# Sweetroll97/GaussianProcessPathModelling

Measured on AMD Instinct MI355X. Metric: gp_fit_predict_points_per_sec, higher is better.
Workload: dtype f64; 1 GPU; C3: exact GP fit+predict, N=65536 d=3 rbf float64, M=4096, inputs resident in HBM; N=65536, d=3, M=4096, kernel=rbf, block=2048, parallelism=1 gpu

## Files before the change

### gaussianprocesspathmodelling_amd/csrc/gpx_api.hip

```cpp
#include <hip/hip_runtime.h>
#include <dlfcn.h>

#include <algorithm>
#include <climits>
#include <cmath>
#include <cstdio>
#include <cstdlib>
#include <cstring>
#include <new>
#include <string>
#include <vector>

#include "../../include/gpx.h"
#include "gpx_cov.h"
#include "gpx_env.h"
#include "gpx_internal.h"

using namespace gpx;

namespace {

thread_local std::string g_create_error;

#define GPX_CATCH_ALL                                  \
  catch (const std::bad_alloc&) { return GPX_E_NOMEM; } \
  catch (...) { return GPX_E_HIP; }

constexpr int RHS_ROWS = 64;

struct Phase {
  hipEvent_t a, b;
  double* target;
};

struct DevBuf {
  void* p = nullptr;
  size_t cap = 0;
  DevBuf() = default;
  DevBuf(DevBuf&& o) noexcept : p(o.p), cap(o.cap) { o.p = nullptr, o.cap = 0; }
  DevBuf& operator=(DevBuf&& o) noexcept {
    std::swap(p, o.p);
    std::swap(cap, o.cap);
    return *this;
  }
  ~DevBuf() {
    if (p) (void)hipFree(p);
  }
};

struct Comm;
struct Group;

}

struct gpx_handle {
  gpx_config cfg{};
  int nb = 1024;
  int nb_solve = 256;
  int nb_pred = 1024;
  EnvKnobs env;
  hipStream_t st = nullptr;
  hipStream_t st2 = nullptr;
  hipStream_t st3 = nullptr;
  hipStream_t st4 = nullptr;
  hipStream_t st5 = nullptr;
  std::string err;
  gpx_timings tm{};
  bool fitted = false;
  int64_t N = 0, Npad = 0, ld = 0, ldp = 0;
  int d = 0, k = 0, n_ls = 1;
  double sf2 = 0, sn2 = 0, jitter = 0;
  double logdet = 0;
  DevBuf X, Xs, ls, K, Winv, P, YT, Y, scalars, info;
  DevBuf var, meanout;
  struct ScratchBufs {
    DevBuf Q, Qs, VT, MT;
    DevBuf Tsol;
    DevBuf MTpart;
    DevBuf ZT, gpart;
    DevBuf ZTloc, ZTpack;
    DevBuf Sv;
// ... 247 lines not shown
    if (seq == 0) HIPCHK(h, hipMemsetAsync(dflag, 0, sizeof(unsigned), s));
    HIPCHK(h, hipEventRecord(e0, s));
    HIPCHK(h, hipStreamWaitEvent(iw->aux, e0, 0));
    HIPCHK(h, hipMemsetAsync(iw->U, 0, (size_t)iw->nbw * iw->ldu * sizeof(T), iw->aux));
    launch_set_diag_one_t<T>(iw->U, iw->ldu, nbp, iw->aux);
    HIPCHK(h, hipMemsetAsync(Wp, 0, (size_t)iw->nbw * iw->nbw * sizeof(T), iw->aux));
  }
  const int diag_step = h->env.diag_step;
  const int nq = nbp / KB;
  for (int q = 0; q < nq;) {
    const int w = (diag_step == 128 && q + 1 < nq) ? 2 : 1;
    const int64_t oq = o + (int64_t)q * KB;
    T* Aqq = A + oq * ld + oq;
    T* Wq = Winv + (oq / KB) * (KB * KB);
    seq += 2;
    if (w == 2)
      launch_potf2_128<T>(Aqq, ld, Wq, gidx0 + oq, info, s, iw && use_flag ? dflag : nullptr, seq);
    else
      launch_potf2_64<T>(Aqq, ld, Wq, gidx0 + oq, info, s, iw && use_flag ? dflag : nullptr, seq);
    const int64_t rem = o + nbp - (oq + w * KB);
    if (rem > 0) {
      T* panel = A + (oq + w * KB) * ld + oq;
      launch_trsm_rlt<T>(panel, ld, rem, Aqq, ld, Wq, w * KB, nullptr, 0, s);
      launch_gemm_nt<T>(64, A + (oq + w * KB) * ld + (oq + w * KB), ld, panel, ld, panel, ld, rem, rem, w * KB, 1, 0, s);
    }
    if (iw) {
      if (use_flag) {
        if (q > 0) {
          launch_wait_counter(dflag, seq - 1, info, iw->aux);
          launch_inv_extend<T>(iw->U, iw->ldu, A + o * ld + o, ld, Winv + (o / KB) * (KB * KB), q, q + w, Wp,
                               iw->nbw, iw->aux, 1);
        }
        launch_wait_counter(dflag, seq, info, iw->aux);
      } else {
        if (int rc = stream_waits(h, iw->aux, s, "block inverse")) return rc;
        launch_inv_extend<T>(iw->U, iw->ldu, A + o * ld + o, ld, Winv + (o / KB) * (KB * KB), q, q + w, Wp, iw->nbw,
                             iw->aux, 1);
      }
      launch_inv_extend<T>(iw->U, iw->ldu, A + o * ld + o, ld, Winv + (o / KB) * (KB * KB), q, q + w, Wp, iw->nbw,
                           iw->aux, 2);
    }
    q += w;
  }
  if (iw) {
    iw->seq = seq;
    if (int rc = record_event(h, iw->aux, "block inverse", &iw->ready)) return rc;
  }
  return GPX_OK;
}

template <typename T>
int panel_solve_enqueue(gpx_handle* h, T* A, int64_t ld, int64_t o, int nbp, int64_t rows_main, int64_t nx,
                        const T* Winv, T* P, int64_t ldp, hipStream_t s, InvWork<T>* iw, int set, int64_t row0 = 0,
                        hipEvent_t prev = nullptr, bool last = true) {
  T* Apanel = A + (o + nbp + row0) * ld + o;
  P += row0 * ldp;
  const int64_t rows = rows_main + nx;
  if (rows <= 0) {
    if (iw && last && row0 > 0) {
      if (int rc = record_event(h, h->st4, "panel copy", &iw->copied[set])) return rc;
    }
    return GPX_OK;
  }
  if (!iw) {
    launch_trsm_rlt<T>(Apanel, ld, rows, A + o * ld + o, ld, Winv + (o / KB) * (KB * KB), nbp, P, ldp, s);
    return GPX_OK;
  }
  const T* Wp = iw->W + (o / iw->nbw) * (int64_t)iw->nbw * iw->nbw;
  HIPCHK(h, hipStreamWaitEvent(s, iw->ready, 0));
  if (row0 == 0 && last) prev = iw->copied[set];
  if (prev) HIPCHK(h, hipStreamWaitEvent(s, prev, 0));
  const int tile_main = gemm_nt_tile((rows_main % 128 == 0 && nbp % 128 == 0) ? 128 : 64, rows_main, nbp, 4);
  if (rows_main > 0 && nx > 0 && tile_main == 64) {
    launch_gemm_nt_fixed<T>(64, P, ldp, Apanel, ld, Wp, iw->nbw, rows, nbp, nbp, 4, 1, s);
  } else {
    if (rows_main > 0) launch_gemm_nt_fixed<T>(tile_main, P, ldp, Apanel, ld, Wp, iw->nbw, rows_main, nbp, nbp, 4, 1, s);
    if (nx > 0)
      launch_gemm_nt<T>(64, P + rows_main * ldp, ldp, Apanel + rows_main * ld, ld, Wp, iw->nbw, nx, nbp, nbp, 4, 1,
                        s);
  }
  if (int rc = stream_waits(h, h->st4, s, "panel copy")) return rc;
  launch_copy2d<T>(Apanel, ld, P, ldp, rows, nbp, h->st4);
  if (last) return record_event(h, h->st4, "panel copy", &iw->copied[set]);
  return GPX_OK;
}

template <typename T>
int chol_enqueue(gpx_handle* h, T* A, int64_t ld, int64_t n, int nb, T* Winv, T* P0, T* P1,
                 int64_t ldp, int* info, int64_t gidx0, bool profile, int64_t nx = 0,
                 InvWork<T>* iw = nullptr, int64_t nx_side = 0) {
  hipStream_t s0 = h->st, s1 = h->st2;
  T* Pbuf[2] = {P0, P1};
  int rc;
  const EnvKnobs& env = h->env;
  const bool fuse_env = fused_strip_in_force(h);
  unsigned* ctr = reinterpret_cast<unsigned*>(info + 8);
  unsigned target = 0;
  auto is_fused = [&](int64_t o) -> bool {
    if (!fuse_env || o >= n) return false;
    const int nbp = (int)std::min<int64_t>(nb, n - o);
    const int64_t ntrail = n - (o + nbp);
    if (ntrail <= 0) return false;
    const int nbn = (int)std::min<int64_t>(nb, ntrail);
    const int64_t nrest = ntrail - nbn;
    if (nrest <= 0 || ntrail % 128 != 0 || nbn % 128 != 0) return false;
    return gemm_nt_tile(128, nrest, nrest, 1) == 128 && gemm_nt_tile(128, ntrail, nbn, 2) == 128;
  };
  auto bordered_update = [&](int64_t o, const T* Pc, hipStream_t s) {
    const int nbp = (int)std::min<int64_t>(nb, n - o);
    const int64_t t0 = o + nbp, ntrail = n - t0;
    if (nx <= 0 || ntrail <= 0) return;
    launch_gemm_nt<T>(nx % 128 == 0 && ntrail % 128 == 0 ? 128 : 64, A + n * ld + t0, ld, Pc + ntrail * ldp, ldp, Pc,
                      ldp, nx, ntrail, nbp, 0, 0, s);
  };
  auto bordered_block = [&](int64_t o, const T* Pc, hipStream_t s, int64_t c0, int64_t nc, int64_t r0, int64_t nr) {
    const int nbp = (int)std::min<int64_t>(nb, n - o);
    const int64_t t0 = o + nbp, ntrail = n - t0;
    if (nr <= 0 || nc <= 0) return;
    launch_gemm_nt<T>(nr % 128 == 0 && nc % 128 == 0 ? 128 : 64, A + (n + r0) * ld + c0, ld, Pc + (ntrail + r0) * ldp, ldp,
                      Pc + (c0 - t0) * ldp, ldp, nr, nc, nbp, 0, 0, s);
  };
  auto update_is_big = [&](int64_t o) -> bool {
    if (o >= n) return false;
    const int nbp = (int)std::min<int64_t>(nb, n - o);
    const int64_t ntrail = n - (o + nbp);
    if (ntrail <= 0) return false;
    const int nbn = (int)std::min<int64_t>(nb, ntrail);
    const int64_t nrest = ntrail - nbn;
    return nrest > 0 && ntrail % 128 == 0 && nbn % 128 == 0 && gemm_nt_tile(128, nrest, nrest, 1) == 128;
  };
  const bool split_env = split_strip_in_force(h);
  const bool top_env = env.solve_top;
  const int rest_split = env.rest_split;
  const int64_t nxs = split_env ? nx_side : 0, nxc = nx - nxs;
  auto side_solve = [&](int64_t o, T* Pp, hipStream_t s) -> int {
    if (nxs <= 0) return GPX_OK;
    const int nbp = (int)std::min<int64_t>(nb, n - o);
    T* Aside = A + (n + nxc) * ld + o;
    T* Pside = Pp + ((n - o - nbp) + nxc) * ldp;
    if (!iw) {
      launch_trsm_rlt<T>(Aside, ld, nxs, A + o * ld + o, ld, Winv + (o / KB) * (KB * KB), nbp, Pside, ldp, s);
      return GPX_OK;
    }
    HIPCHK(h, hipStreamWaitEvent(s, iw->ready, 0));
    launch_gemm_nt<T>(nxs % 128 == 0 && nbp % 128 == 0 ? 128 : 64, Pside, ldp, Aside, ld,
                      iw->W + (o / iw->nbw) * (int64_t)iw->nbw * iw->nbw, iw->nbw, nxs, nbp, nbp, 4, 1, s);
    launch_copy2d<T>(Aside, ld, Pside, ldp, nxs, nbp, s);
    return GPX_OK;
  };
  LatencyGuard latency_guard;
  set_latency_mode(1);
  const int resv_k = env.cu_self_reserve;
  ReserveGuard reserve_guard;
  if (resv_k > 0 && split_env) {
    if ((rc = ensure(h, h->resv_ring, (size_t)RESV_RING * 8 * sizeof(unsigned)))) return rc;
    HIPCHK(h, hipMemsetAsync(h->resv_ring.p, 0, (size_t)RESV_RING * 8 * sizeof(unsigned), s0));
    reserve_ring((unsigned*)h->resv_ring.p, RESV_RING, env.resv_form);
  }
  const bool any_fused = is_fused(0);
  if (any_fused) HIPCHK(h, hipMemsetAsync(ctr, 0, sizeof(unsigned), s0));
  {
    const int nb0 = (int)std::min<int64_t>(nb, n);
    {
      PhaseScope ps(h, &h->tm.chol_diag, profile);
      if ((rc = diag_enqueue(h, A, ld, 0, nb0, Winv, info, gidx0, s0, iw))) return rc;
    }
    {
      PhaseScope ps(h, &h->tm.chol_trsm, profile);
      if ((rc = panel_solve_enqueue(h, A, ld, 0, nb0, n - nb0, nxc, Winv, Pbuf[0], ldp, s0, iw, 0))) return rc;
    }
    if (any_fused) {
      bordered_update(0, Pbuf[0], s0);
      if ((rc = stream_waits(h, s1, s0, "look-ahead"))) return rc;
    }
  }
  hipEvent_t e_main = nullptr;
  if (split_env && n > nb && (rc = record_event(h, s0, "look-ahead", &e_main))) return rc;
  int step = 0;
  for (int64_t o = 0; o < n; o += nb, ++step) {
    const int nbp = (int)std::min<int64_t>(nb, n - o);
    const int64_t t0 = o + nbp;
    const int64_t ntrail = n - t0;
    if (ntrail <= 0) {
      if ((rc = side_solve(o, Pbuf[step & 1], s0))) return rc;
      break;
    }
    T* Pc = Pbuf[step & 1];
    T* Pn = Pbuf[(step + 1) & 1];
    const int nbn = (int)std::min<int64_t>(nb, ntrail);
    const int64_t nrest = ntrail - nbn;
    const int tile = (ntrail % 128 == 0 && nbn % 128 == 0) ? 128 : 64;
    hipEvent_t e_panel = next_event(h);
    if (!e_panel) return fail(h, GPX_E_HIP, "hipEventCreate failed (look-ahead)");
    set_latency_mode(update_is_big(o) ? 0 : 1);
    if (is_fused(o)) {
      {
        PhaseScope ps(h, &h->tm.chol_syrk, profile);
        target += launch_gemm_nt_fused<T>(A + t0 * ld + t0, ld, Pc, ldp, ntrail, nbn, nbp, ctr, s0);
        h->tm.syrk_flops += (double)ntrail * (double)(ntrail + 1) * (double)nbp;
        h->tm.syrk_launches += 1;
      }
      launch_wait_counter(ctr, target, info, s1);
      {
        PhaseScope ps(h, &h->tm.chol_diag, profile, s1);
        if ((rc = diag_enqueue(h, A, ld, t0, nbn, Winv, info, gidx0, s1, iw))) return rc;
      }
      {
        PhaseScope ps(h, &h->tm.chol_trsm, profile, s1);
        if ((rc = panel_solve_enqueue(h, A, ld, t0, nbn, nrest, nx, Winv, Pn, ldp, s1, iw, (step + 1) & 1))) return rc;
      }
      HIPCHK(h, hipEventRecord(e_panel, s1));
      if (is_fused(t0)) bordered_update(t0, Pn, s1);
      HIPCHK(h, hipStreamWaitEvent(s0, e_panel, 0));
      continue;
    }
    if (split_env) {
      hipStream_t sm = s0;
      const int resv_it = (resv_k > 0 && (env.resv_all || ntrail <= (int64_t)(rest_split + 1) * nb)) ? resv_k : 0;
      if (e_main) HIPCHK(h, hipStreamWaitEvent(s1, e_main, 0));
      {
        PhaseScope ps(h, &h->tm.chol_strip, profile, s1);
        launch_gemm_nt<T>(tile, A + t0 * ld + t0, ld, Pc, ldp, Pc, ldp, nbn, nbn, nbp, 1, 0, s1);
      }
      set_reserve_mode(resv_it);
      {
        PhaseScope ps(h, &h->tm.chol_strip, profile, sm);
        if (nrest > 0)
          launch_gemm_nt<T>(tile, A + (t0 + nbn) * ld + t0, ld, Pc + (int64_t)nbn * ldp, ldp, Pc, ldp, nrest, nbn, nbp, 0,
                            0, sm);
        bordered_block(o, Pc, sm, t0, nbn, 0, nxc);
      }
      hipEvent_t e_below;
      if ((rc = record_event(h, sm, "look-ahead", &e_below))) return rc;
      const int nbn2 = (int)std::min<int64_t>(nb, nrest);
      const bool ahead = nrest > nbn2 && nrest <= (int64_t)rest_split * nb;
      T* Cr = A + (t0 + nbn) * ld + (t0 + nbn);
      const T* Pr = Pc + (int64_t)nbn * ldp;
      if (ahead) {
        {
          PhaseScope ps(h, &h->tm.chol_strip, profile, sm);
          launch_gemm_nt<T>(tile, Cr, ld, Pr, ldp, Pr, ldp, nrest, nbn2, nbp, 2, 0, sm);
        }
        if ((rc = record_event(h, sm, "look-ahead", &e_main))) return rc;
      }
      const int64_t nr = ahead ? nrest - nbn2 : nrest, off = ahead ? nbn2 : 0;
      if (nr > 0) {
        const bool big = gemm_nt_tile(tile, nr, nr, 1) == 128;
        PhaseScope ps(h, big ? &h->tm.chol_syrk : &h->tm.chol_strip, profile, sm);
        launch_gemm_nt<T>(tile, Cr + off * ld + off, ld, Pr + off * ldp, ldp, Pr + off * ldp, ldp, nr, nr, nbp, 1, 0, sm);
        if (big) {
          h->tm.syrk_flops += (double)nr * (double)(nr + 1) * (double)nbp;
          h->tm.syrk_launches += 1;
        }
      }
      if (!ahead && (rc = record_event(h, sm, "look-ahead", &e_main))) return rc;
      {
        PhaseScope ps(h, &h->tm.chol_strip, profile, sm);
        bordered_block(o, Pc, sm, t0 + nbn, nrest, 0, nxc);
        if ((rc = side_solve(o, Pc, sm))) return rc;
        bordered_block(o, Pc, sm, t0, ntrail, nxc, nxs);
      }
      set_reserve_mode(0);
      {
        PhaseScope ps(h, &h->tm.chol_diag, profile, s1);
        set_reserve_chain(resv_it > 0 ? env.resv_chain : 0);
        rc = diag_enqueue(h, A, ld, t0, nbn, Winv, info, gidx0, s1, iw);
        set_reserve_chain(0);
        if (rc) return rc;
      }
      HIPCHK(h, hipStreamWaitEvent(s1, e_below, 0));
      const int64_t top = (iw && top_env) ? std::min<int64_t>(nrest, nb) : nrest;
      hipEvent_t prev_copied = iw ? iw->copied[(step + 1) & 1] : nullptr;
      {
        PhaseScope ps(h, &h->tm.chol_trsm, profile, s1);
        if (top < nrest || (iw && top_env)) {
          if ((rc = panel_solve_enqueue(h, A, ld, t0, nbn, top, 0, Winv, Pn, ldp, s1, iw, (step + 1) & 1, 0, prev_copied,
                                        false)))
            return rc;
        } else if ((rc = panel_solve_enqueue(h, A, ld, t0, nbn, nrest, nxc, Winv, Pn, ldp, s1, iw, (step + 1) & 1))) {
          return rc;
        }
      }
      HIPCHK(h, hipEventRecord(e_panel, s1));
      HIPCHK(h, hipStreamWaitEvent(sm, e_panel, 0));
      if (top < nrest || (iw && top_env)) {
        PhaseScope ps(h, &h->tm.chol_trsm, profile, sm);
        set_reserve_mode(resv_it);
        rc = panel_solve_enqueue(h, A, ld, t0, nbn, nrest - top, nxc, Winv, Pn, ldp, sm, iw, (step + 1) & 1, top, prev_copied,
                                 true);
        set_reserve_mode(0);
        if (rc) return rc;
      }
      continue;
    }
    {
      PhaseScope ps(h, &h->tm.chol_strip, profile);
      set_latency_mode(1);
      launch_gemm_nt<T>(tile, A + t0 * ld + t0, ld, Pc, ldp, Pc, ldp, ntrail, nbn, nbp, 2, 0, s0);
      set_latency_mode(update_is_big(o) ? 0 : 1);
      bordered_update(o, Pc, s0);
    }
    if ((rc = stream_waits(h, s1, s0, "look-ahead"))) return rc;
    {
      {
        PhaseScope ps(h, &h->tm.chol_diag, profile, s1);
        if ((rc = diag_enqueue(h, A, ld, t0, nbn, Winv, info, gidx0, s1, iw))) return rc;
      }
      {
        PhaseScope ps(h, &h->tm.chol_trsm, profile, s1);
        if ((rc = panel_solve_enqueue(h, A, ld, t0, nbn, nrest, nx, Winv, Pn, ldp, s1, iw, (step + 1) & 1))) return rc;
      }
    }
    HIPCHK(h, hipEventRecord(e_panel, s1));
    if (nrest > 0) {
      const bool big = gemm_nt_tile(tile, nrest, nrest, 1) == 128;
      PhaseScope ps(h, big ? &h->tm.chol_syrk : &h->tm.chol_strip, profile);
      launch_gemm_nt<T>(tile, A + (t0 + nbn) * ld + (t0 + nbn), ld, Pc + (int64_t)nbn * ldp, ldp,
                        Pc + (int64_t)nbn * ldp, ldp, nrest, nrest, nbp, 1, 0, s0);
      if (big) {
        h->tm.syrk_flops += (double)nrest * (double)(nrest + 1) * (double)nbp;
        h->tm.syrk_launches += 1;
      }
    }
    HIPCHK(h, hipStreamWaitEvent(s0, e_panel, 0));
  }
  if (iw) {
    for (hipStream_t sj : {iw->aux, h->st4})
      if ((rc = stream_waits(h, s0, sj, "join"))) return rc;
  }
  return GPX_OK;
}

template <typename T>
struct SolveWork {
  const T* W = nullptr;
  int nbw = 0;
  T *T0 = nullptr, *T1 = nullptr;
  int64_t ldt = 0;
};

template <typename T>
int solve_fwd_enqueue(gpx_handle* h, T* XT, int64_t rows, const T* L, int64_t ld, int64_t n, int nb,
                      const T* Winv, const SolveWork<T>* wb = nullptr) {
  hipStream_t s0 = h->st, s1 = h->st2;
  const int tile = (rows % 128 == 0) ? 128 : 64;
  LatencyGuard latency_guard;
  set_latency_mode(1);
  if (rows < 128 || !s1) {
    for (int64_t o = 0; o < n; o += nb) {
      const int nbp = (int)std::min<int64_t>(nb, n - o);
      launch_trsm_rlt<T>(XT + o, ld, rows, L + o * ld + o, ld, Winv + (o / KB) * (KB * KB), nbp, nullptr,
                         0, s0);
      const int64_t ntrail = n - (o + nbp);
      if (ntrail > 0)
        launch_gemm_nt<T>((ntrail % 128 == 0) ? tile : 64, XT + o + nbp, ld, XT + o, ld,
                          L + (o + nbp) * ld + o, ld, rows, ntrail, nbp, 0, 0, s0);
    }
    return GPX_OK;
  }
  const bool dense = wb && wb->nbw == nb && wb->T0 && h->st4;
  T* Ts[2] = {dense ? wb->T0 : nullptr, dense ? wb->T1 : nullptr};
  hipEvent_t e_copy[2] = {nullptr, nullptr};
  const int64_t ldt = dense ? wb->ldt : 0;
// ... 143 lines not shown

template <typename T>
int dense_solve_work(gpx_handle* h, DevBuf& buf, int64_t rows, SolveWork<T>* sw) {
  if (h->nbw != h->nb_pred || (h->comm && !h->repl)) return GPX_OK;
  int rc;
  sw->ldt = h->nbw + ld_skew<T>();
  if ((rc = ensure(h, buf, (size_t)2 * rows * sw->ldt * sizeof(T)))) return rc;
  sw->W = (const T*)h->Wblk.p;
  sw->nbw = h->nbw;
  sw->T0 = (T*)buf.p;
  sw->T1 = sw->T0 + rows * sw->ldt;
  return GPX_OK;
}

template <typename T>
void mean_product(gpx_handle* h, T* MT, int64_t ldm, const T* rhsT, const T* VT, int64_t cols, T* part, int64_t ldpart) {
  const int ksplit = splitk_splits(h->Npad);
  if (ksplit > 1)
    launch_gemm_nt_splitk<T>(MT, ldm, rhsT, h->ld, VT, h->ld, RHS_ROWS, cols, h->Npad, ksplit, part, ldpart, h->st);
  else
    launch_gemm_nt<T>(64, MT, ldm, rhsT, h->ld, VT, h->ld, RHS_ROWS, cols, h->Npad, 0, 1, h->st);
}

template <typename T>
int ensure_mean_partials(gpx_handle* h, DevBuf& part, int64_t ldpart) {
  const int ksplit = splitk_splits(h->Npad);
  return ksplit > 1 ? ensure(h, part, (size_t)ksplit * RHS_ROWS * ldpart * sizeof(T)) : GPX_OK;
}

template <typename T>
void bordered_mean_var(gpx_handle* h, const T* VT, int64_t rows, int64_t rows_pad, int64_t ldm, bool want_var) {
  {
    PhaseScope ps(h, &h->tm.mean);
    mean_product<T>(h, (T*)h->scr.MT.p, ldm, (const T*)h->zT, VT, rows_pad, (T*)h->scr.MTpart.p, ldm);
    launch_unpack_rhs<T>((const T*)h->scr.MT.p, ldm, rows, h->k, 1.0, (T*)h->meanout.p, h->st);
  }
  if (want_var) {
    PhaseScope ps(h, &h->tm.var);
    launch_var_rows<T>(VT, h->ld, rows, h->Npad, h->sf2, (T*)h->var.p, h->st);
  }
}

template <typename T>
int deliver_mean_var(gpx_handle* h, void* mean, void* var, int64_t M, int32_t mem_kind) {
  PhaseScope ps(h, &h->tm.d2h);
  int rc;
  if ((rc = copy_out(h, mean, h->meanout.p, (size_t)M * h->k * sizeof(T), mem_kind))) return rc;
  return var ? copy_out(h, var, h->var.p, (size_t)M * sizeof(T), mem_kind) : GPX_OK;
}

template <typename T>
int predict_core(gpx_handle* h, const void* Xq, int64_t M, bool want_var, int32_t mem_kind);
bool few_solver_applies(const gpx_handle* h);
template <typename T>
int solve_few(gpx_handle* h, T* RT, int k, const T* L, int64_t ld, int64_t n, const T* W, int nb, bool forward = true,
              bool backward = true);

}

#include "gpx_shard.inc"
#include "gpx_group.inc"

namespace {

template <typename T>
int stage_fit_weights(gpx_handle* h, int64_t N, int64_t cap) {
  h->weighted = false;
  if (h->nw_set == 0) return GPX_OK;
  int rc;
  if ((rc = ensure(h, h->Wfit, (size_t)cap * sizeof(T)))) return rc;
  if (h->cfg.dtype == GPX_MIXED) {
    if ((rc = ensure(h, h->Wfit64, (size_t)cap * 8))) return rc;
    HIPCHK(h, hipMemcpyAsync(h->Wfit64.p, h->Wset.p, (size_t)N * 8, hipMemcpyDeviceToDevice, h->st));
    launch_f64_to_f32((const double*)h->Wfit64.p, (float*)h->Wfit.p, N, h->st);
  } else {
    HIPCHK(h, hipMemcpyAsync(h->Wfit.p, h->Wset.p, (size_t)N * sizeof(T), hipMemcpyDeviceToDevice, h->st));
  }
  h->weighted = true;
  return GPX_OK;
}

template <typename T>
int fit_impl(gpx_handle* h, const void* X, const void* y, int64_t N, int32_t d, int32_t k,
             const double* lengthscale, int32_t n_ls, double sf2, double sn2, double jitter,
             int32_t mem_kind, int64_t* info, const void* Xq = nullptr, int64_t M = 0, bool retried = false) {
  const int64_t Npad = round_up(N, TILE);
  const int64_t Mpad = Xq ? round_up(M, TILE) : 0;
  const int64_t cap = h->reserve > 0 ? std::max(Npad, round_up(h->reserve, TILE)) : Npad;
  const int64_t capN = h->reserve > 0 ? cap : N;
  const int64_t ld = cap + ld_skew<T>();
  if (h->cfg.block == 0) {
    h->nb = auto_panel_width(h, Npad);
    if (h->env.nb_pred < 0) h->nb_pred = h->nb;
  }
  const int64_t ldp = h->nb + ld_skew<T>();
  h->N = N; h->Npad = Npad; h->ld = ld; h->ldp = ldp; h->d = d; h->k = k; h->n_ls = n_ls;
  h->sf2 = sf2; h->sn2 = sn2; h->jitter = jitter;
  const bool profile = (h->cfg.flags & GPX_FLAG_PROFILE) != 0;
  gpx_timings& tm = h->tm;
  tm.h2d = tm.kbuild = tm.chol = tm.solve = tm.logdet = tm.fit_total = 0;
  tm.chol_diag = tm.chol_trsm = tm.chol_strip = tm.chol_syrk = tm.syrk_flops = tm.comm = 0;
  tm.syrk_launches = 0;
  tm.kbuild_bytes = (double)sizeof(T) * ((double)N * (double)(N + 1) / 2.0 + (double)N * d);

  int rc;
  if ((rc = flag_handover_probe(h))) return rc;
  if ((rc = ensure(h, h->X, (size_t)capN * d * sizeof(T)))) return rc;
  if ((rc = ensure(h, h->Y, (size_t)capN * k * sizeof(T)))) return rc;
  if ((rc = ensure(h, h->Xs, (size_t)cap * d * sizeof(T)))) return rc;
  if ((rc = ensure(h, h->ls, MAX_D * 8))) return rc;
  const int64_t NX = RHS_ROWS + Mpad;
  if (Xq && (rc = ensure_queries<T>(h, M))) return rc;
  if ((rc = ensure(h, h->K, (size_t)(cap + NX) * ld * sizeof(T)))) return rc;
  if ((rc = ensure(h, h->Winv, (size_t)(cap / KB) * KB * KB * sizeof(T)))) return rc;
  if ((rc = ensure(h, h->P, (size_t)2 * (cap + NX) * ldp * sizeof(T)))) return rc;
  if ((rc = ensure(h, h->scalars, 64))) return rc;
  if ((rc = ensure(h, h->info, 64))) return rc;
  const int64_t nblk = (cap + h->nb - 1) / h->nb;
  const int64_t ldu = h->nb + ld_skew<T>();
  if ((rc = ensure(h, h->Wblk, (size_t)nblk * h->nb * h->nb * sizeof(T)))) return rc;
  if ((rc = ensure(h, h->Ublk, (size_t)h->nb * ldu * sizeof(T)))) return rc;
  if ((rc = stage_fit_weights<T>(h, N, cap))) return rc;
  InvWork<T> iw;
  iw.W = (T*)h->Wblk.p;
  iw.U = (T*)h->Ublk.p;
  iw.ldu = ldu;
  iw.nbw = h->nb;
  iw.aux = h->st3;
  h->nbw = 0;

  T* dK = (T*)h->K.p;
  h->Lfac = dK;
  h->repl = false;
  T* dYT = dK + Npad * ld;
  h->zT = dYT;
  h->alphaT = nullptr;
  h->alpha_ready = false;
  int* dInfo = (int*)h->info.p;
  {
    PhaseScope total(h, &tm.fit_total);
    {
      PhaseScope ps(h, &tm.h2d);
      if ((rc = copy_in(h, h->X.p, X, (size_t)N * d * sizeof(T), mem_kind))) return rc;
      if ((rc = copy_in(h, h->Y.p, y, (size_t)N * k * sizeof(T), mem_kind))) return rc;
      if ((rc = copy_in(h, h->ls.p, lengthscale, (size_t)n_ls * 8, GPX_MEM_HOST))) return rc;
      const int init = INT_MAX;
      HIPCHK(h, hipMemcpyAsync(dInfo, &init, sizeof(int), hipMemcpyHostToDevice, h->st));
    }
    {
      PhaseScope ps(h, &tm.kbuild);
      launch_scale_points<T>((const T*)h->X.p, N, Npad, d, (const double*)h->ls.p, n_ls,
                          (T*)h->Xs.p, h->st);
      if (h->weighted)
        launch_kbuild_sym_w<T>(h->cfg.kernel, (const T*)h->Xs.p, N, Npad, d, sf2, (const T*)h->Wfit.p, sn2, jitter, dK, ld,
                               h->st);
      else
        launch_kbuild_sym<T>(h->cfg.kernel, (const T*)h->Xs.p, N, Npad, d, sf2, sn2 + jitter, dK, ld, h->st);
      if (Xq) {
        if ((rc = upload_queries<T>(h, Xq, M, mem_kind))) return rc;
        launch_kbuild_cross<T>(h->cfg.kernel, (const T*)h->scr.Qs.p, M, Mpad, (const T*)h->Xs.p, N, Npad, d, sf2,
                            dK + (Npad + RHS_ROWS) * ld, ld, h->st);
      }
    }
    {
      PhaseScope ps(h, &tm.chol);
      launch_pack_rhs<T>((const T*)h->Y.p, N, k, dYT, ld, Npad, RHS_ROWS, h->st);
      if ((rc = chol_enqueue<T>(h, dK, ld, Npad, h->nb, (T*)h->Winv.p, (T*)h->P.p,
                                (T*)h->P.p + (Npad + NX) * ldp, ldp, dInfo, 0, profile, NX, &iw, Mpad)))
        return rc;
    }
    {
      PhaseScope ps(h, &tm.logdet);
      launch_logdet<T>(dK, ld, Npad, (double*)h->scalars.p, h->st);
    }
  }
  int hinfo = 0;
  HIPCHK(h, hipMemcpyAsync(&hinfo, dInfo, sizeof(int), hipMemcpyDeviceToHost, h->st));
  HIPCHK(h, hipMemcpyAsync(&h->logdet, h->scalars.p, sizeof(double), hipMemcpyDeviceToHost, h->st));
  if ((rc = finish_call(h))) return rc;
  if (hinfo < 0) {
    if (retry_with_events(h, retried))
      return fit_impl<T>(h, X, y, N, d, k, lengthscale, n_ls, sf2, sn2, jitter, mem_kind, info, Xq, M, true);
    return fail(h, GPX_E_HIP,
                "a stream parked on a device flag timed out: kernels are being serialised across streams — "
                "set GPX_CHAIN_FLAG=0 (and leave GPX_FUSED_STRIP unset) to hand over by hipEvents instead");
  }
  tm.handover_flags = chain_flag_enabled(h) ? 1.0 : 0.0;
  tm.handover_retries = (double)h->flag_retries;
  *info = (hinfo == INT_MAX) ? 0 : (int64_t)hinfo;
  h->fitted = (*info == 0);
  if (h->fitted) h->nbw = h->nb;
  return GPX_OK;
}


template <typename T>
int append_room(gpx_handle* h, int64_t Nnew, bool with_weights) {
  const int64_t skew = ld_skew<T>(), cap0 = h->ld - skew, NpadNew = round_up(Nnew, TILE), want = round_up(h->reserve, TILE);
  const int64_t N = h->N, Npad = h->Npad, nb = h->nb, d = h->d, k = h->k;
  const bool relayout = NpadNew > cap0 || want > cap0;
  const int64_t cap = !relayout ? cap0 : NpadNew <= want ? want : round_up(Nnew + nb, TILE);
  const int64_t ld = cap + skew, R0 = N / nb * nb;
  struct Grow {
    DevBuf* buf;
    size_t need, keep;
    DevBuf fresh;
  } g[] = {{&h->X, (size_t)cap * d * sizeof(T), (size_t)N * d * sizeof(T), {}},
           {&h->Y, (size_t)cap * k * sizeof(T), (size_t)N * k * sizeof(T), {}},
           {&h->Xs, (size_t)cap * d * sizeof(T), (size_t)Npad * d * sizeof(T), {}},
           {&h->Winv, (size_t)(cap / KB) * KB * KB * sizeof(T), (size_t)(Npad / KB) * KB * KB * sizeof(T), {}},
           {&h->Wblk, (size_t)((cap + nb - 1) / nb) * nb * nb * sizeof(T), (size_t)(R0 / nb) * nb * nb * sizeof(T), {}},
           {&h->Wfit, with_weights ? (size_t)cap * sizeof(T) : 0, h->weighted ? (size_t)N * sizeof(T) : 0, {}}};
  const size_t kbytes = (size_t)(cap + RHS_ROWS) * ld * sizeof(T);
  const size_t pbytes = (size_t)2 * (cap + RHS_ROWS) * h->ldp * sizeof(T);
  const bool newK = relayout || h->K.cap < kbytes, newP = h->P.cap < pbytes;
  double need = (newK ? (double)kbytes : 0.0) + (newP ? (double)pbytes : 0.0);
  for (Grow& x : g)
    if (x.buf->cap < x.need) need += (double)x.need;
  if (need == 0.0) return GPX_OK;
  size_t freeb = 0, totalb = 0;
  HIPCHK(h, hipMemGetInfo(&freeb, &totalb));
  const double avail = (double)freeb + (newP ? (double)h->P.cap : 0.0);
// ... 152 lines not shown
                    "a stream parked on a device flag timed out: kernels are being serialised across streams — "
                    "set GPX_CHAIN_FLAG=0 (and leave GPX_FUSED_STRIP unset) to hand over by hipEvents instead");
      if ((r = begin_call(h))) return r;
    }
  };
  int hinfo = 0;
  if ((rc = restart(Nnew, Xnew, ynew, &hinfo))) return rc;
  *info = (hinfo == INT_MAX) ? 0 : (int64_t)hinfo;
  int64_t Nfit = Nnew;
  if (*info > 0) {
    int back = 0;
    if ((rc = begin_call(h))) return rc;
    if ((rc = restart(Nold, nullptr, nullptr, &back))) return rc;
    if (back != INT_MAX) return fail(h, GPX_E_HIP, "gpx_append: the previous fit could not be restored");
    Nfit = Nold;
    h->weighted = was_weighted;
  }
  h->N = Nfit;
  h->Npad = round_up(Nfit, TILE);
  tm.handover_flags = chain_flag_enabled(h) ? 1.0 : 0.0;
  tm.handover_retries = (double)h->flag_retries;
  h->fitted = true;
  return GPX_OK;
}

template <typename T>
int solve_few(gpx_handle* h, T* RT, int k, const T* L, int64_t ld, int64_t n, const T* W, int nbw, bool forward, bool backward) {
  const int nb = std::min(nbw, 1024);
  auto Wsub = [&](int64_t o) -> const T* {
    return W + (o / nbw) * (int64_t)nbw * nbw + ((o % nbw) / nb) * ((int64_t)nb * nbw + nb);
  };
  int rc;
  if ((rc = ensure(h, h->Zfew, (size_t)8 * nb * sizeof(T)))) return rc;
  T* Zs = (T*)h->Zfew.p;
  hipStream_t st = h->st;
  for (int64_t o = 0; forward && o < n; o += nb) {
    const int nbp = (int)std::min<int64_t>(nb, n - o);
    const int64_t t0 = o + nbp;
    launch_few_product<T>(false, true, Zs, nb, Wsub(o), nbw, nbp, nbp, RT + o, ld, k, st);
    HIPCHK(h, hipMemcpy2DAsync(RT + o, (size_t)ld * sizeof(T), Zs, (size_t)nb * sizeof(T), (size_t)nbp * sizeof(T), k,
                               hipMemcpyDeviceToDevice, st));
    launch_few_product<T>(false, false, RT + t0, ld, L + t0 * ld + o, ld, n - t0, nbp, Zs, nb, k, st);
  }
  for (int64_t o = ((n - 1) / nb) * nb; backward && o >= 0; o -= nb) {
    const int nbp = (int)std::min<int64_t>(nb, n - o);
    launch_few_product<T>(true, true, Zs, nb, Wsub(o), nbw, nbp, nbp, RT + o, ld, k, st);
    HIPCHK(h, hipMemcpy2DAsync(RT + o, (size_t)ld * sizeof(T), Zs, (size_t)nb * sizeof(T), (size_t)nbp * sizeof(T), k,
                               hipMemcpyDeviceToDevice, st));
    launch_few_product<T>(true, false, RT, ld, L + o * ld, ld, o, nbp, Zs, nb, k, st);
  }
  return GPX_OK;
}

bool few_solver_applies(const gpx_handle* h) {
  return h->env.few_solve && h->nbw > 0 && (h->nbw <= 1024 ? h->nbw % 128 == 0 : h->nbw % 1024 == 0) && h->k <= 8 &&
         (!h->comm || h->repl) && h->Wblk.p;
}

template <typename T>
int ensure_alpha(gpx_handle* h) {
  if (h->alpha_ready) return GPX_OK;
  int rc;
  if ((rc = ensure(h, h->AT, (size_t)RHS_ROWS * h->ld * sizeof(T)))) return rc;
  PhaseScope ps(h, &h->tm.solve);
  HIPCHK(h, hipMemcpyAsync(h->AT.p, h->zT, (size_t)RHS_ROWS * h->ld * sizeof(T), hipMemcpyDeviceToDevice,
                           h->st));
  if (few_solver_applies(h)) {
    if ((rc = solve_few<T>(h, (T*)h->AT.p, h->k, (const T*)h->Lfac, h->ld, h->Npad, (const T*)h->Wblk.p, h->nbw, false)))
      return rc;
  } else
    solve_bwd_enqueue<T>(h, (T*)h->AT.p, RHS_ROWS, (const T*)h->Lfac, h->ld, h->Npad, h->nb_solve,
                         (const T*)h->Winv.p);
  h->alphaT = h->AT.p;
  h->alpha_ready = true;
  return GPX_OK;
}

template <typename T>
int predict_core(gpx_handle* h, const void* Xq, int64_t M, bool want_var, int32_t mem_kind) {
  if (M <= 0) return GPX_OK;
  const int64_t N = h->N, Npad = h->Npad, ld = h->ld;
  const int d = h->d, k = h->k;
  const int64_t Mpad = round_up(M, TILE);
  const int64_t ldm = Mpad + ld_skew<T>();
  const int64_t MB = pred_batch_rows(h, Mpad, (size_t)ld * sizeof(T), true);
  gpx_timings& tm = h->tm;
  int rc;
  if ((rc = ensure_queries<T>(h, M))) return rc;
  if ((rc = ensure(h, h->scr.VT, (size_t)MB * ld * sizeof(T)))) return rc;
  if ((rc = ensure(h, h->scr.MT, (size_t)RHS_ROWS * ldm * sizeof(T)))) return rc;
  const int64_t ldpm = std::min(MB, Mpad) + ld_skew<T>();
  if ((rc = ensure_mean_partials<T>(h, h->scr.MTpart, ldpm))) return rc;
  if ((rc = ensure(h, h->meanout, (size_t)M * k * sizeof(T)))) return rc;
  if ((rc = ensure(h, h->var, (size_t)Mpad * sizeof(T)))) return rc;
  SolveWork<T> sw;
  if (want_var && (rc = dense_solve_work<T>(h, h->scr.Tsol, MB, &sw))) return rc;
  T* dVT = (T*)h->scr.VT.p;
  const T* dK = (const T*)h->Lfac;
  const T* dWinv = (const T*)h->Winv.p;
  if (!want_var && (rc = ensure_alpha<T>(h))) return rc;
  const T* rhsT = (const T*)(want_var ? h->zT : h->alphaT);
  {
    PhaseScope ps(h, &tm.kstar);
    if ((rc = upload_queries<T>(h, Xq, M, mem_kind))) return rc;
  }
  for (int64_t m0 = 0; m0 < Mpad; m0 += MB) {
    const int64_t mp = std::min(MB, Mpad - m0);
    const int64_t mv = std::min<int64_t>(mp, M - m0);
    {
      PhaseScope ps(h, &tm.kstar);
// ... 1771 lines not shown
```

### gaussianprocesspathmodelling_amd/csrc/gpx_env.h

```cpp
#ifndef GPX_ENV_H_
#define GPX_ENV_H_

#include <cstdint>
#include <cstdio>
#include <cstdlib>
#include <cstring>

namespace gpx {

enum class EnvAt { create, call, process };

namespace env_rule {
inline bool flag(const char* e) { return atoi(e) != 0; }
inline int block(const char* e, int hi, int otherwise) {
  const int v = atoi(e);
  return (v >= 128 && v <= hi && v % 128 == 0) ? v : otherwise;
}
inline int64_t in_range(int64_t v, int64_t lo, int64_t hi, int64_t otherwise) { return (v >= lo && v <= hi) ? v : otherwise; }
}

#define GPX_ENV_TABLE(X)                                                                                               \
                                                               \
  X("GPX_DIAG_STEP", diag_step, Int, call, 128, atoi(e) == 64 ? 64 : 128)                                              \
  X("GPX_CHAIN_FLAG", chain_flag, Opt, call, -1, env_rule::flag(e))                                                    \
  X("GPX_FUSED_STRIP", fused_strip, Flag, call, false, env_rule::flag(e))                                              \
  X("GPX_SPLIT_STRIP", split_strip, Flag, call, true, env_rule::flag(e))                                               \
  X("GPX_SOLVE_TOP", solve_top, Flag, call, true, env_rule::flag(e))                                                   \
  X("GPX_REST_SPLIT", rest_split, Int, call, 16, atoi(e))                                                              \
  X("GPX_CU_SELF_RESERVE", cu_self_reserve, Int, call, 0, (int)env_rule::in_range(atoi(e), 1, 4, 0))                   \
  X("GPX_RESV_ALL", resv_all, Flag, call, false, env_rule::flag(e))                                                    \
  X("GPX_RESV_CHAIN", resv_chain, Int, call, 1, atoi(e))                                                               \
  X("GPX_RESV_FORM", resv_form, Int, call, 1, atoi(e))                                                                 \
                                                                                               \
  X("GPX_NB_WIDE_FROM", nb_wide_from, I64, call, 40960, (int64_t)atoll(e))                                             \
  X("GPX_NB_GRAD", nb_grad, Int, call, 0, env_rule::block(e, 4096, 0))                                                 \
  X("GPX_NB_SOLVE", nb_solve, Int, create, 256, env_rule::block(e, 4096, 256))                                         \
  X("GPX_NB_PRED", nb_pred, Opt, create, -1, env_rule::block(e, 4096, 1024))                                           \
  X("GPX_NB_SHARD", nb_shard, Int, create, 0, env_rule::block(e, 2048, 0))                                             \
  X("GPX_PRED_BATCH", pred_batch, I64, call, 8192, env_rule::in_range(atol(e), 128, 1L << 22, 8192) / 128 * 128)       \
  X("GPX_FEW_SOLVE", few_solve, Flag, call, true, env_rule::flag(e))                                                   \
                                                                                         \
  X("GPX_SHARD_DEAL", shard_snake, Int, call, 1, (strcmp(e, "cyclic") == 0 || strcmp(e, "0") == 0) ? 0 : 1)            \
  X("GPX_SHARD_REPLICATE", shard_replicate, Opt, call, -1, env_rule::flag(e))                                          \
  X("GPX_SHARD_DENSE_PANEL", shard_dense_panel, Flag, call, true, env_rule::flag(e))                                   \
  X("GPX_SHARD_TWO_PIPE", shard_two_pipe, Opt, call, -1, env_rule::flag(e))                                            \
  X("GPX_SHARD_FUSED", shard_fused, Flag, call, true, env_rule::flag(e))                                               \
  X("GPX_REPL_COPY_SIDE", repl_copy_side, Flag, call, true, env_rule::flag(e))                                         \
  X("GPX_GROUP_INITALL", group_initall, Flag, call, true, env_rule::flag(e))                                           \
  X("GPX_LOCAL_FORCE_PEER", local_force_peer, Flag, call, false, env_rule::flag(e))                                    \
                                                                                                      \
  X("GPX_MICROBENCH_ITERS", microbench_iters, Int, call, 65536, (int)env_rule::in_range(atol(e), 64, 1L << 20, 65536)) \
  X("GPX_ROCTX", roctx, Flag, process, true, env_rule::flag(e))                                                        \
  X("GPX_RCCL_PATH", rccl_path, Str, process, nullptr, e)

struct EnvKnobs {
  using Flag = bool;
  using Int = int;
  using I64 = int64_t;
  using Opt = int;
  using Str = const char*;
#define GPX_ENV_FIELD(name, field, kind, at, dflt, rule) kind field = dflt;
  GPX_ENV_TABLE(GPX_ENV_FIELD)
#undef GPX_ENV_FIELD
  bool counters_collected = false;
};

inline void env_read(EnvKnobs& k, EnvAt at) {
#define GPX_ENV_READ(name, field, kind, at_, dflt, rule) \
  if (at == EnvAt::at_) {                                \
    const char* e = getenv(name);                        \
    k.field = e ? (rule) : (dflt);                       \
  }
  GPX_ENV_TABLE(GPX_ENV_READ)
#undef GPX_ENV_READ
  if (at == EnvAt::call) {
    const char* e = getenv("ROCPROF_COUNTER_COLLECTION");
    k.counters_collected = e && atoi(e) != 0;
  }
}

inline int env_print(const EnvKnobs& k, char* buf, int n) {
// ... 21 lines not shown
```

Baseline: 43770 points/s.

## Solve packed RHS rows after Cholesky instead of bordering them through factorization

For large problems, the packed right-hand-side rows (RHS_ROWS of the bordered block) are excluded from the bordered trailing updates and panel solves during the blocked Cholesky. The forward solve for them then runs afterwards with the few-RHS block-inverse solver. The intent is to stop carrying those extra rows through every panel GEMM and copy, and replace that with one separate triangular solve pass. A new env knob (GPX_RHS_RIDE) can force either path. The default uses the new path when Npad is at least 16384 and the few-solver applies.

```diff
diff --git a/gaussianprocesspathmodelling_amd/csrc/gpx_api.hip b/gaussianprocesspathmodelling_amd/csrc/gpx_api.hip
--- a/gaussianprocesspathmodelling_amd/csrc/gpx_api.hip
+++ b/gaussianprocesspathmodelling_amd/csrc/gpx_api.hip
@@ -27,6 +27,7 @@
   catch (...) { return GPX_E_HIP; }
 
 constexpr int RHS_ROWS = 64;
+constexpr int64_t RHS_AFTER_FROM = 16384;
 
 struct Phase {
   hipEvent_t a, b;
@@ -380,9 +381,10 @@
 template <typename T>
 int panel_solve_enqueue(gpx_handle* h, T* A, int64_t ld, int64_t o, int nbp, int64_t rows_main, int64_t nx,
                         const T* Winv, T* P, int64_t ldp, hipStream_t s, InvWork<T>* iw, int set, int64_t row0 = 0,
-                        hipEvent_t prev = nullptr, bool last = true) {
+                        hipEvent_t prev = nullptr, bool last = true, int64_t nx0 = 0) {
   T* Apanel = A + (o + nbp + row0) * ld + o;
   P += row0 * ldp;
+  if (nx <= 0) nx0 = 0;
   const int64_t rows = rows_main + nx;
   if (rows <= 0) {
     if (iw && last && row0 > 0) {
@@ -391,7 +393,14 @@
     return GPX_OK;
   }
   if (!iw) {
-    launch_trsm_rlt<T>(Apanel, ld, rows, A + o * ld + o, ld, Winv + (o / KB) * (KB * KB), nbp, P, ldp, s);
+    if (nx0 == 0) {
+      launch_trsm_rlt<T>(Apanel, ld, rows, A + o * ld + o, ld, Winv + (o / KB) * (KB * KB), nbp, P, ldp, s);
+    } else {
+      if (rows_main > 0)
+        launch_trsm_rlt<T>(Apanel, ld, rows_main, A + o * ld + o, ld, Winv + (o / KB) * (KB * KB), nbp, P, ldp, s);
+      launch_trsm_rlt<T>(Apanel + (rows_main + nx0) * ld, ld, nx, A + o * ld + o, ld, Winv + (o / KB) * (KB * KB), nbp,
+                         P + (rows_main + nx0) * ldp, ldp, s);
+    }
     return GPX_OK;
   }
   const T* Wp = iw->W + (o / iw->nbw) * (int64_t)iw->nbw * iw->nbw;
@@ -399,16 +408,21 @@
   if (row0 == 0 && last) prev = iw->copied[set];
   if (prev) HIPCHK(h, hipStreamWaitEvent(s, prev, 0));
   const int tile_main = gemm_nt_tile((rows_main % 128 == 0 && nbp % 128 == 0) ? 128 : 64, rows_main, nbp, 4);
-  if (rows_main > 0 && nx > 0 && tile_main == 64) {
+  if (rows_main > 0 && nx > 0 && nx0 == 0 && tile_main == 64) {
     launch_gemm_nt_fixed<T>(64, P, ldp, Apanel, ld, Wp, iw->nbw, rows, nbp, nbp, 4, 1, s);
   } else {
     if (rows_main > 0) launch_gemm_nt_fixed<T>(tile_main, P, ldp, Apanel, ld, Wp, iw->nbw, rows_main, nbp, nbp, 4, 1, s);
     if (nx > 0)
-      launch_gemm_nt<T>(64, P + rows_main * ldp, ldp, Apanel + rows_main * ld, ld, Wp, iw->nbw, nx, nbp, nbp, 4, 1,
-                        s);
+      launch_gemm_nt<T>(64, P + (rows_main + nx0) * ldp, ldp, Apanel + (rows_main + nx0) * ld, ld, Wp, iw->nbw, nx, nbp,
+                        nbp, 4, 1, s);
   }
   if (int rc = stream_waits(h, h->st4, s, "panel copy")) return rc;
-  launch_copy2d<T>(Apanel, ld, P, ldp, rows, nbp, h->st4);
+  if (nx0 == 0) {
+    launch_copy2d<T>(Apanel, ld, P, ldp, rows, nbp, h->st4);
+  } else {
+    if (rows_main > 0) launch_copy2d<T>(Apanel, ld, P, ldp, rows_main, nbp, h->st4);
+    launch_copy2d<T>(Apanel + (rows_main + nx0) * ld, ld, P + (rows_main + nx0) * ldp, ldp, nx, nbp, h->st4);
+  }
   if (last) return record_event(h, h->st4, "panel copy", &iw->copied[set]);
   return GPX_OK;
 }
@@ -416,7 +430,7 @@
 template <typename T>
 int chol_enqueue(gpx_handle* h, T* A, int64_t ld, int64_t n, int nb, T* Winv, T* P0, T* P1,
                  int64_t ldp, int* info, int64_t gidx0, bool profile, int64_t nx = 0,
-                 InvWork<T>* iw = nullptr, int64_t nx_side = 0) {
+                 InvWork<T>* iw = nullptr, int64_t nx_side = 0, int64_t nx_idle = 0) {
   hipStream_t s0 = h->st, s1 = h->st2;
   T* Pbuf[2] = {P0, P1};
   int rc;
@@ -438,8 +452,9 @@
     const int nbp = (int)std::min<int64_t>(nb, n - o);
     const int64_t t0 = o + nbp, ntrail = n - t0;
     if (nx <= 0 || ntrail <= 0) return;
-    launch_gemm_nt<T>(nx % 128 == 0 && ntrail % 128 == 0 ? 128 : 64, A + n * ld + t0, ld, Pc + ntrail * ldp, ldp, Pc,
-                      ldp, nx, ntrail, nbp, 0, 0, s);
+    const int tile = gemm_nt_tile(nx % 128 == 0 && ntrail % 128 == 0 ? 128 : 64, nx, ntrail, 0);
+    launch_gemm_nt_fixed<T>(tile, A + (n + nx_idle) * ld + t0, ld, Pc + (ntrail + nx_idle) * ldp, ldp, Pc, ldp, nx - nx_idle,
+                            ntrail, nbp, 0, 0, s);
   };
   auto bordered_block = [&](int64_t o, const T* Pc, hipStream_t s, int64_t c0, int64_t nc, int64_t r0, int64_t nr) {
     const int nbp = (int)std::min<int64_t>(nb, n - o);
@@ -461,6 +476,8 @@
   const bool top_env = env.solve_top;
   const int rest_split = env.rest_split;
   const int64_t nxs = split_env ? nx_side : 0, nxc = nx - nxs;
+  if (nx_idle < 0 || nx_idle > nxc || nx_idle % KB != 0) return fail(h, GPX_E_ARG, "chol_enqueue: bad count of idle bordered rows");
+  const int64_t nxr = nxc - nx_idle;
   auto side_solve = [&](int64_t o, T* Pp, hipStream_t s) -> int {
     if (nxs <= 0) return GPX_OK;
     const int nbp = (int)std::min<int64_t>(nb, n - o);
@@ -495,7 +512,8 @@
     }
     {
       PhaseScope ps(h, &h->tm.chol_trsm, profile);
-      if ((rc = panel_solve_enqueue(h, A, ld, 0, nb0, n - nb0, nxc, Winv, Pbuf[0], ldp, s0, iw, 0))) return rc;
+      if ((rc = panel_solve_enqueue(h, A, ld, 0, nb0, n - nb0, nxr, Winv, Pbuf[0], ldp, s0, iw, 0, 0, nullptr, true, nx_idle)))
+        return rc;
     }
     if (any_fused) {
       bordered_update(0, Pbuf[0], s0);
@@ -535,7 +553,9 @@
       }
       {
         PhaseScope ps(h, &h->tm.chol_trsm, profile, s1);
-        if ((rc = panel_solve_enqueue(h, A, ld, t0, nbn, nrest, nx, Winv, Pn, ldp, s1, iw, (step + 1) & 1))) return rc;
+        if ((rc = panel_solve_enqueue(h, A, ld, t0, nbn, nrest, nxr, Winv, Pn, ldp, s1, iw, (step + 1) & 1, 0, nullptr, true,
+                                      nx_idle)))
+          return rc;
       }
       HIPCHK(h, hipEventRecord(e_panel, s1));
       if (is_fused(t0)) bordered_update(t0, Pn, s1);
@@ -556,7 +576,7 @@
         if (nrest > 0)
           launch_gemm_nt<T>(tile, A + (t0 + nbn) * ld + t0, ld, Pc + (int64_t)nbn * ldp, ldp, Pc, ldp, nrest, nbn, nbp, 0,
                             0, sm);
-        bordered_block(o, Pc, sm, t0, nbn, 0, nxc);
+        bordered_block(o, Pc, sm, t0, nbn, nx_idle, nxr);
       }
       hipEvent_t e_below;
       if ((rc = record_event(h, sm, "look-ahead", &e_below))) return rc;
@@ -584,7 +604,7 @@
       if (!ahead && (rc = record_event(h, sm, "look-ahead", &e_main))) return rc;
       {
         PhaseScope ps(h, &h->tm.chol_strip, profile, sm);
-        bordered_block(o, Pc, sm, t0 + nbn, nrest, 0, nxc);
+        bordered_block(o, Pc, sm, t0 + nbn, nrest, nx_idle, nxr);
         if ((rc = side_solve(o, Pc, sm))) return rc;
         bordered_block(o, Pc, sm, t0, ntrail, nxc, nxs);
       }
@@ -605,7 +625,8 @@
           if ((rc = panel_solve_enqueue(h, A, ld, t0, nbn, top, 0, Winv, Pn, ldp, s1, iw, (step + 1) & 1, 0, prev_copied,
                                         false)))
             return rc;
-        } else if ((rc = panel_solve_enqueue(h, A, ld, t0, nbn, nrest, nxc, Winv, Pn, ldp, s1, iw, (step + 1) & 1))) {
+        } else if ((rc = panel_solve_enqueue(h, A, ld, t0, nbn, nrest, nxr, Winv, Pn, ldp, s1, iw, (step + 1) & 1, 0, nullptr,
+                                             true, nx_idle))) {
           return rc;
         }
       }
@@ -614,8 +635,8 @@
       if (top < nrest || (iw && top_env)) {
         PhaseScope ps(h, &h->tm.chol_trsm, profile, sm);
         set_reserve_mode(resv_it);
-        rc = panel_solve_enqueue(h, A, ld, t0, nbn, nrest - top, nxc, Winv, Pn, ldp, sm, iw, (step + 1) & 1, top, prev_copied,
-                                 true);
+        rc = panel_solve_enqueue(h, A, ld, t0, nbn, nrest - top, nxr, Winv, Pn, ldp, sm, iw, (step + 1) & 1, top, prev_copied,
+                                 true, nx_idle);
         set_reserve_mode(0);
         if (rc) return rc;
       }
@@ -636,7 +657,9 @@
       }
       {
         PhaseScope ps(h, &h->tm.chol_trsm, profile, s1);
-        if ((rc = panel_solve_enqueue(h, A, ld, t0, nbn, nrest, nx, Winv, Pn, ldp, s1, iw, (step + 1) & 1))) return rc;
+        if ((rc = panel_solve_enqueue(h, A, ld, t0, nbn, nrest, nxr, Winv, Pn, ldp, s1, iw, (step + 1) & 1, 0, nullptr, true,
+                                      nx_idle)))
+          return rc;
       }
     }
     HIPCHK(h, hipEventRecord(e_panel, s1));
@@ -886,6 +909,7 @@
 template <typename T>
 int predict_core(gpx_handle* h, const void* Xq, int64_t M, bool want_var, int32_t mem_kind);
 bool few_solver_applies(const gpx_handle* h);
+bool few_solver_takes(const gpx_handle* h, int nbw);
 template <typename T>
 int solve_few(gpx_handle* h, T* RT, int k, const T* L, int64_t ld, int64_t n, const T* W, int nb, bool forward = true,
               bool backward = true);
@@ -971,6 +995,8 @@
   h->alphaT = nullptr;
   h->alpha_ready = false;
   int* dInfo = (int*)h->info.p;
+  const bool rhs_after =
+      h->env.rhs_ride != 1 && few_solver_takes(h, h->nb) && (h->env.rhs_ride == 0 || Npad >= RHS_AFTER_FROM);
   {
     PhaseScope total(h, &tm.fit_total);
     {
@@ -1000,8 +1026,13 @@
       PhaseScope ps(h, &tm.chol);
       launch_pack_rhs<T>((const T*)h->Y.p, N, k, dYT, ld, Npad, RHS_ROWS, h->st);
       if ((rc = chol_enqueue<T>(h, dK, ld, Npad, h->nb, (T*)h->Winv.p, (T*)h->P.p,
-                                (T*)h->P.p + (Npad + NX) * ldp, ldp, dInfo, 0, profile, NX, &iw, Mpad)))
+                                (T*)h->P.p + (Npad + NX) * ldp, ldp, dInfo, 0, profile, NX, &iw, Mpad,
+                                rhs_after ? RHS_ROWS : 0)))
         return rc;
+    }
+    if (rhs_after) {
+      PhaseScope ps(h, &tm.solve);
+      if ((rc = solve_few<T>(h, dYT, k, dK, ld, Npad, (const T*)h->Wblk.p, h->nb, true, false))) return rc;
     }
     {
       PhaseScope ps(h, &tm.logdet);
@@ -1260,10 +1291,11 @@
   return GPX_OK;
 }
 
-bool few_solver_applies(const gpx_handle* h) {
-  return h->env.few_solve && h->nbw > 0 && (h->nbw <= 1024 ? h->nbw % 128 == 0 : h->nbw % 1024 == 0) && h->k <= 8 &&
+bool few_solver_takes(const gpx_handle* h, int nbw) {
+  return h->env.few_solve && nbw > 0 && (nbw <= 1024 ? nbw % 128 == 0 : nbw % 1024 == 0) && h->k <= 8 &&
          (!h->comm || h->repl) && h->Wblk.p;
 }
+bool few_solver_applies(const gpx_handle* h) { return few_solver_takes(h, h->nbw); }
 
 template <typename T>
 int ensure_alpha(gpx_handle* h) {
diff --git a/gaussianprocesspathmodelling_amd/csrc/gpx_env.h b/gaussianprocesspathmodelling_amd/csrc/gpx_env.h
--- a/gaussianprocesspathmodelling_amd/csrc/gpx_env.h
+++ b/gaussianprocesspathmodelling_amd/csrc/gpx_env.h
@@ -27,6 +27,7 @@
   X("GPX_SPLIT_STRIP", split_strip, Flag, call, true, env_rule::flag(e))                                               \
   X("GPX_SOLVE_TOP", solve_top, Flag, call, true, env_rule::flag(e))                                                   \
   X("GPX_REST_SPLIT", rest_split, Int, call, 16, atoi(e))                                                              \
+  X("GPX_RHS_RIDE", rhs_ride, Opt, call, -1, env_rule::flag(e))                                                        \
   X("GPX_CU_SELF_RESERVE", cu_self_reserve, Int, call, 0, (int)env_rule::in_range(atoi(e), 1, 4, 0))                   \
   X("GPX_RESV_ALL", resv_all, Flag, call, false, env_rule::flag(e))                                                    \
   X("GPX_RESV_CHAIN", resv_chain, Int, call, 1, atoi(e))                                                               \
```

Result: no change. 43940 points/s, median of 6 (+0.4%).
